# pangsu0613/TransCAR

Hardware: AMD Instinct MI355X
Metric: nuScenes frames/sec (6-cam+radar, 900 queries): fusion decoder (Detr3DHead.forward + box decode), FPN features resident in HBM (higher is better)
Workload: dtype f32 (linear steps and attention core of the batched launches: f16x2 split operands, 3 v_mfma_f32_16x16x32_f16 products, fp32 accumulate; activations of the 32-row tiles held as two f16 planes; 4- / 8-row tiles: f32 MFMA)

## Files before the change

transcar_amd/csrc/head.hip:

```cpp
#include <math.h>
#include <stdarg.h>
#include <stdlib.h>
#include <string.h>

#include "kernels.hpp"

namespace tc {

static thread_local char g_err[512] = "";

void set_error(const char* fmt, ...) {
  va_list ap;
  va_start(ap, fmt);
  vsnprintf(g_err, sizeof(g_err), fmt, ap);
  va_end(ap);
}

int check_launch(const char* what) {
  hipError_t e = hipGetLastError();
  if (e != hipSuccess) {
    set_error("%s: %s", what, hipGetErrorString(e));
    return (int)e;
  }
  return 0;
// ... 55 lines not shown
                             int np = 1) {
  const int rows = B * Q;
  const int NL = ncams * feats->num_levels * np;
  TC_TRY(linear(query, C, aw, rows, C, NL, 0, ws.logits, NL, s, pos));
  CamSampleArgs c;
  c.feats = *feats; c.B = B; c.Q = Q; c.C = C; c.num_cams = ncams; c.num_points = np;
  c.lidar2img = l2i; c.ref = ref; c.logits = ws.logits;
  for (int i = 0; i < 6; ++i) c.pc[i] = pc[i];
  c.img_h = img_h; c.img_w = img_w; c.out = ws.sampled; c.vis = nullptr; c.pair_counter = pair_counter;
  TC_TRY(launch_cam_sample(c, s));
  TC_TRY(linear(ws.sampled, C, oproj, rows, C, C, 0, ws.t0, C, s, nullptr, query, C));
  TC_TRY(launch_posenc_l1(ref, 3, 1, pe.l0.w, pe.l0.b, pe.n1.g, pe.n1.b, ws.pe0, rows, s));
  return linear(ws.pe0, C, pe.l3, rows, C, C, 0, ws.pe1, C, s);
}

static int head_points(const tc_head_weights* w) { return w->num_points > 0 ? w->num_points : 1; }

static int check_dims(const tc_head_weights* w) {
  TC_REQUIRE(w != nullptr, "weights pointer is null");
  TC_REQUIRE(w->abi_version == TC_ABI_VERSION, "tc_head_weights.abi_version=%d, library=%d",
             w->abi_version, TC_ABI_VERSION);
  TC_REQUIRE(w->embed_dims == 256 && w->num_heads == 8, "embed_dims=%d num_heads=%d (256/8 supported)",
             w->embed_dims, w->num_heads);
  TC_REQUIRE(w->num_layers >= 1 && w->num_layers <= TC_MAX_LAYERS, "num_layers=%d", w->num_layers);
  TC_REQUIRE(w->num_radar_layers >= 0 && w->num_radar_layers <= TC_MAX_RADAR_LAYERS,
             "num_radar_layers=%d", w->num_radar_layers);
  TC_REQUIRE(w->num_levels == 4, "num_levels=%d (4 supported)", w->num_levels);
  TC_REQUIRE(w->num_points >= 0 && w->num_cams * w->num_levels * head_points(w) <= TC_MAX_CAM_LOGITS,
             "num_points=%d (num_cams * num_levels * num_points <= %d supported)", w->num_points, TC_MAX_CAM_LOGITS);
  TC_REQUIRE((w->ffn_dims & 31) == 0 && (w->radar_in_dims & 3) == 0, "ffn_dims/radar_in_dims alignment");
  return 0;
}

static int decoder_refines(const tc_head_weights* w, bool* refine) {
  const int L = w->num_layers;
  const bool r = L < 2 || w->layers[0].reg.l0.w != nullptr;
  for (int l = 1; l + 1 < L; ++l)
    TC_REQUIRE((w->layers[l].reg.l0.w != nullptr) == r,
               "layers[%d].reg is %s but layers[0].reg is %s: below the last layer the reg branches are all set (box "
               "refinement) or all NULL (none)", l, r ? "NULL" : "set", r ? "set" : "NULL");
  TC_REQUIRE(w->layers[L - 1].reg.l0.w != nullptr, "layers[%d].reg is NULL: the last layer's reg branch "
             "(reg_branches[-1]) is required with and without box refinement", L - 1);
  *refine = r;
  return 0;
}

struct HeadWs {
  float *pos, *x, *qk, *vt, *attn_o, *t0, *t1, *t2, *ffn_h, *logits, *sampled;
  float *init_ref, *inter_refs, *hs, *reg_tmp, *box_m;
  float *tp0, *tp1, *f0, *f1, *f2, *radar_feat, *kv, *qproj, *rattn, *cxy, *addref, *qf;
  float* kv3[TC_MAX_RADAR_LAYERS];
  int* hits;
  int *perm, *hitflag;
  int qpad;
};

static size_t head_ws_layout(const tc_head_weights* w, int B, int T, void* base, size_t cap,
                             HeadWs* out) {
  const int Q = w->num_query, C = w->embed_dims, F = w->ffn_dims, L = w->num_layers;
  const size_t rows = (size_t)B * Q, rt = (size_t)B * T;
  const int qpad = ((Q + 15) / 16) * 16;
  Arena a(base, cap);
  HeadWs h;
  h.qpad = qpad;
  h.pos = a.take<float>(rows * C); h.x = a.take<float>(rows * C);
  h.qk = a.take<float>(rows * 2 * C); h.vt = a.take<float>((size_t)B * C * qpad);
  h.attn_o = a.take<float>(rows * C);
  h.t0 = a.take<float>(rows * C); h.t1 = a.take<float>(rows * C); h.t2 = a.take<float>(rows * C);
  h.ffn_h = a.take<float>(rows * F);
  h.logits = a.take<float>(rows * w->num_cams * w->num_levels * head_points(w));
  h.sampled = a.take<float>(rows * C);
  h.init_ref = a.take<float>(rows * 3); h.inter_refs = a.take<float>((size_t)L * rows * 3);
  h.hs = a.take<float>((size_t)L * rows * C);
  h.reg_tmp = a.take<float>(rows * w->code_size); h.box_m = a.take<float>(rows * w->code_size);
  h.tp0 = a.take<float>(rt * C); h.tp1 = a.take<float>(rt * C);
  h.f0 = a.take<float>(rt * 64); h.f1 = a.take<float>(rt * 128); h.f2 = a.take<float>(rt * C);
  h.radar_feat = a.take<float>(rt * C); h.kv = a.take<float>(rt * 2 * C);
  for (int i = 0; i < TC_MAX_RADAR_LAYERS; ++i) h.kv3[i] = a.take<float>(rt * 2 * C);
  h.qproj = a.take<float>(rows * C); h.rattn = a.take<float>(rows * C);
  h.cxy = a.take<float>(rows * 2); h.addref = a.take<float>(rows * 3);
  h.qf = a.take<float>(rows * C);
  h.hits = a.take<int>((size_t)TC_MAX_RADAR_LAYERS * rows);
  h.perm = a.take<int>(rows); h.hitflag = a.take<int>(rows);
  if (out) *out = h;
  return a.off;
}

static int head_forward_fused(const tc_head_weights* w, const tc_feats_nhwc* feats, int B,
                              const float* lidar2img, float img_h, float img_w,
                              const float* radar_tokens, int T, int pad_mult, float* all_cls_scores,
                              float* all_bbox_preds, const tc_head_aux* aux, const tc_head_options& opt,
                              const HeadWs& h_, hipStream_t s) {
  const int Q = w->num_query, C = w->embed_dims, L = w->num_layers, H = w->num_heads;
  const int code = w->code_size, ncls = w->num_classes;
  const int rows = B * Q, rt = B * T;
  const float attn_qscale = 1.4426950408889634f / sqrtf((float)(C / H));
  HeadWs h = h_;
  if (aux != nullptr) {
    if (aux->inter_states) h.hs = aux->inter_states;
    if (aux->inter_references) h.inter_refs = aux->inter_references;
    if (aux->last_box) h.box_m = aux->last_box;
  }
  unsigned long long* pairs = aux ? aux->sample_pairs : nullptr;
  const bool radar = w->num_radar_layers > 0;
  bool refine = true;
  TC_TRY(decoder_refines(w, &refine));

  const int enc_first = opt.phase != 0 && L > 1 ? L - 2 : 0;
  const int lid_begin = opt.phase == 2 ? enc_first : 0, lid_end = opt.phase == 1 ? enc_first : L;
  RadarEncodeArgs re;
  if (radar) {
    re.tokens = radar_tokens; re.RI = w->radar_in_dims; re.M = rt;
    re.rpe = w->radar_position_encoder; re.f0 = w->radar_feat0; re.f2 = w->radar_feat2;
    re.f4 = w->radar_feat4; re.nlayers = w->num_radar_layers;
    for (int r = 0; r < TC_MAX_RADAR_LAYERS; ++r) {
      const tc_mha& m = w->radar[r].attn;
      re.kvproj[r] = tc_linear{m.in_proj.w ? m.in_proj.w + (size_t)C * C : nullptr,
                               m.in_proj.b ? m.in_proj.b + C : nullptr};
      re.kv[r] = h.kv3[r];
    }
    re.radar_feat = h.radar_feat;
    re.w16_delta = w->packed16_delta; re.matrix_path = opt.matrix_path; re.range_status = opt.range_status;
  }

  const bool ddrop = opt.decoder_dropout_p > 0.0f;
  TC_REQUIRE(!ddrop || (unsigned long long)(opt.dropout_seed_stride ? 1 : B) * H * Q * Q < (1ull << 32),
             "decoder dropout: B*H*Q*Q exceeds 32 bits");
  if (radar && ddrop && opt.phase != 1) TC_TRY(launch_radar_encode(re, s));
  const bool folded = !ddrop && w->l0_attn_out != nullptr && w->l0_init_reference != nullptr;
  if (!folded && opt.phase != 2) {
    PrologueArgs pa;
    pa.qe = w->query_embedding; pa.Q = Q; pa.M = rows; pa.refpts = w->reference_points;
    pa.in_proj = w->layers[0].self_attn.in_proj; pa.init_ref = h.init_ref; pa.qk = h.qk; pa.vt = h.vt;
    pa.qpad = h.qpad; pa.qscale = attn_qscale; pa.w16_delta = w->packed16_delta;
    TC_TRY(launch_prologue(pa, s));
  }
  for (int lid = lid_begin; lid < lid_end; ++lid) {
    const bool l0c = folded && lid == 0;
    const bool init_in = lid == 0 || !refine;
    const float* ref_in = init_in ? (folded ? w->l0_init_reference : h.init_ref)
                                  : h.inter_refs + (size_t)(lid - 1) * rows * 3;
    DecoderChainArgs d;
    if (ddrop) {
      d.drop = make_drop(opt.decoder_dropout_p, opt.dropout_seed, 16u + 8u * (unsigned)lid, 0u);
      if (opt.dropout_seed_stride != 0) { d.drop.seed_stride = opt.dropout_seed_stride; d.drop.rows_per_sample = (unsigned)Q; }
    }
    d.attn_o = l0c ? w->l0_attn_out : h.attn_o;
    d.attn_mod = l0c ? Q : 0; d.ref_mod = folded && init_in ? Q : 0;
    if (lid == 0) { d.x_in = w->query_embedding + C; d.x_ld = 2 * C; d.x_mod = Q; }
    else { d.x_in = h.hs + (size_t)(lid - 1) * rows * C; d.x_ld = C; d.x_mod = 0; }
    d.qe = w->query_embedding; d.Q = Q;
    d.ref_in = ref_in; d.ref_out = h.inter_refs + (size_t)lid * rows * 3;
    d.box_m = lid == L - 1 ? h.box_m : nullptr;
    if (!refine) d.ref_out = h.addref;
    d.w = &w->layers[lid];
    d.next_in_proj = lid + 1 < L ? &w->layers[lid + 1].self_attn.in_proj : nullptr;
    d.qscale = attn_qscale;
    d.hs = h.hs + (size_t)lid * rows * C; d.qk = h.qk; d.vt = h.vt; d.qpad = h.qpad;
    d.cam.feats = *feats; d.cam.B = B; d.cam.Q = Q; d.cam.C = C; d.cam.num_cams = w->num_cams;
    d.cam.num_points = head_points(w);
    d.cam.lidar2img = lidar2img; d.cam.ref = ref_in; d.cam.logits = nullptr;
    for (int i = 0; i < 6; ++i) d.cam.pc[i] = w->pc_range[i];
    d.cam.img_h = img_h; d.cam.img_w = img_w; d.cam.out = nullptr; d.cam.vis = nullptr;
    d.cam.pair_counter = pairs;
    d.code = code; d.M = rows; d.tile_rows = opt.chain_tile_rows; d.matrix_path = opt.matrix_path;
    d.range_status = opt.range_status;
    if (!l0c) {
      const int trows = opt.chain_tile_rows ? opt.chain_tile_rows : (rows <= 1024 ? 4 : rows <= 2048 ? 8 : 16);
      if (trows >= 16 && opt.matrix_path != TC_MATRIX_F32) {
        PreGatherArgs pga;
        const bool pre = !ddrop && opt.cam_pregather == 1;
        if (pre) {
          float* pbuf = static_cast<float*>(opt.cam_pregather_ws);
          int* pmask = reinterpret_cast<int*>(pbuf + (size_t)rows * w->num_cams * w->num_levels * C);
          pga.cam = d.cam; pga.M = rows; pga.ref_mod = d.ref_mod; pga.out = pbuf; pga.mask = pmask;
          d.pre = pbuf; d.premask = pmask;
        }
        TC_TRY(launch_self_attn_core_x(h.qk, h.qk + C, 2 * C, h.vt, h.qpad, h.attn_o, C, B, Q, H, s, ddrop ? &d.drop : nullptr,
                                       pre ? &pga : nullptr));
      } else {
        TC_TRY(launch_self_attn_core(h.qk, h.qk + C, 2 * C, h.vt, h.qpad, h.attn_o, C, B, Q, H, s, ddrop ? &d.drop : nullptr));
      }
    }
    if (radar && !ddrop && lid == enc_first) TC_TRY(launch_decoder_chain_with_encoders(d, re, L > 1 ? 1 : 0, s));
    else if (radar && !ddrop && L > 1 && lid == enc_first + 1) TC_TRY(launch_decoder_chain_with_encoders(d, re, 2, s));
    else TC_TRY(launch_decoder_chain(d, s));
  }
  if (opt.phase == 1) return 0;
  if (!refine)
    TC_TRY(launch_ref_broadcast(folded ? w->l0_init_reference : h.init_ref, folded ? Q : 0, h.inter_refs, rows, L, s));
  if (aux) {
    if (aux->init_reference) {
      if (folded) {
        for (int b = 0; b < B; ++b)
          TC_HIP(hipMemcpyAsync(aux->init_reference + (size_t)b * Q * 3, w->l0_init_reference,
                                (size_t)Q * 3 * 4, hipMemcpyDeviceToDevice, s));
      } else {
        TC_HIP(hipMemcpyAsync(aux->init_reference, h.init_ref, (size_t)rows * 3 * 4, hipMemcpyDeviceToDevice, s));
      }
    }
  }
  if (!radar) return 0;
  RadarChainArgs rc;
  rc.qf = h.hs + (size_t)(L - 1) * rows * C;
  rc.ref_last = h.inter_refs + (size_t)(L - 1) * rows * 3;
  rc.box_m = h.box_m; rc.tokens = radar_tokens; rc.RI = w->radar_in_dims;
  for (int r = 0; r < TC_MAX_RADAR_LAYERS; ++r) { rc.kv[r] = h.kv3[r]; rc.w[r] = w->radar[r]; }
  rc.nlayers = w->num_radar_layers; rc.Q = Q; rc.T = T; rc.pad_mult = pad_mult; rc.code = code;
  rc.ncls = ncls; rc.M = rows; rc.qscale = 1.0f / sqrtf((float)(C / H));
  for (int i = 0; i < 6; ++i) rc.pc[i] = w->pc_range[i];
  rc.all_cls = all_cls_scores; rc.all_box = all_bbox_preds; rc.hits = h.hits;
  rc.tile_rows = opt.chain_tile_rows; rc.last_cls_only = opt.last_level_cls_only; rc.matrix_path = opt.matrix_path;
  rc.range_status = opt.range_status;
  if (opt.radar_row_order == 2 || (opt.radar_row_order == 0 && rows > 1024)) {
    TC_TRY(launch_radar_compact(rc.ref_last, rc.box_m, code, 0, w->pc_range, radar_tokens, w->radar_in_dims, B, Q, T,
                                w->radar[0].radius_min, w->radar[0].radius_max, h.hitflag, h.perm, s));
    rc.row_perm = h.perm;
  }
  TC_TRY(launch_radar_chain(rc, s));
  if (aux && aux->radar_hit_counts)
    TC_HIP(hipMemcpyAsync(aux->radar_hit_counts, h.hits, (size_t)w->num_radar_layers * rows * 4,
                          hipMemcpyDeviceToDevice, s));
  return 0;
}

struct PackItem { const float* src; int N, K; const float** slot; bool narrow; bool absent; };

static int collect_pack_items(const tc_head_weights* w, tc_head_weights* v, PackItem* it) {
  const int C = w->embed_dims, F = w->ffn_dims, NL = w->num_cams * w->num_levels * head_points(w);
  const int code = w->code_size, ncls = w->num_classes;
  int n = 0;
  auto add = [&](const tc_linear& src, tc_linear& dst, int N, int K, bool narrow = false, bool absent = false) {
// ... 175 lines not shown
size_t tc_self_attn_workspace_bytes(int B, int Q, int C) {
  const size_t rows = (size_t)B * Q;
  const size_t qpad = ((Q + 15) / 16) * 16;
  return arena_slice(rows * 2 * C, 4) + arena_slice((size_t)B * C * qpad, 4) + arena_slice(rows * C, 4);
}

int tc_self_attn_fwd(const tc_mha* w, const float* x, const float* pos, float* out, int B, int Q,
                     int C, int num_heads, void* workspace, size_t workspace_bytes,
                     tc_stream_t stream) {
  TC_REQUIRE(C == 256 && num_heads == 8, "self_attn: C=%d heads=%d (256/8 supported)", C, num_heads);
  TC_REQUIRE(workspace_bytes >= tc_self_attn_workspace_bytes(B, Q, C), "self_attn: workspace too small");
  const size_t rows = (size_t)B * Q;
  const int qpad = ((Q + 15) / 16) * 16;
  Arena a(workspace, workspace_bytes);
  float* qk = a.take<float>(rows * 2 * C);
  float* vt = a.take<float>((size_t)B * C * qpad);
  float* ao = a.take<float>(rows * C);
  return self_attn(*w, x, pos, out, B, Q, C, num_heads, qk, vt, qpad, ao, as_stream(stream));
}

int tc_decoder_layer_tail_fwd(const tc_decoder_layer* layer, const tc_linear* next_in_proj,
                              const tc_feats_nhwc* feats, int B, int Q, int num_cams,
                              int code_size, const float* attn_o, const float* x_in,
                              const float* query_embedding, const float* lidar2img,
                              const float* ref_in, const float* pc_range, float img_h,
                              float img_w, float* hs, float* ref_out, float* qk, float* vt,
                              int qpad, int tile_rows, tc_stream_t stream) {
  TC_REQUIRE(layer != nullptr && feats != nullptr, "decoder_layer_tail: null argument");
  const int C = 256;
  DecoderChainArgs d;
  d.attn_o = attn_o; d.x_in = x_in; d.x_ld = C; d.x_mod = 0;
  d.qe = query_embedding; d.Q = Q; d.ref_in = ref_in; d.ref_out = ref_out; d.box_m = nullptr;
  d.w = layer; d.next_in_proj = next_in_proj;
  d.qscale = 1.4426950408889634f / sqrtf(32.0f);
  d.hs = hs; d.qk = qk; d.vt = vt; d.qpad = qpad;
  d.cam.feats = *feats; d.cam.B = B; d.cam.Q = Q; d.cam.C = C; d.cam.num_cams = num_cams;
  d.cam.lidar2img = lidar2img; d.cam.ref = ref_in; d.cam.logits = nullptr;
  for (int i = 0; i < 6; ++i) d.cam.pc[i] = pc_range[i];
  d.cam.img_h = img_h; d.cam.img_w = img_w; d.cam.out = nullptr; d.cam.vis = nullptr;
  d.cam.pair_counter = nullptr;
  d.code = code_size; d.M = B * Q; d.tile_rows = TC_TILE_ROWS(tile_rows); d.matrix_path = TC_TILE_MATRIX(tile_rows);
  TC_REQUIRE(d.matrix_path <= TC_MATRIX_F16X2 && (tile_rows >> 10) == 0, "decoder_layer_tail: tile_rows=0x%x", tile_rows);
  TC_TRY(launch_decoder_chain(d, as_stream(stream)));
  if (layer->reg.l0.w == nullptr)
    TC_HIP(hipMemcpyAsync(ref_out, ref_in, (size_t)B * Q * 3 * 4, hipMemcpyDeviceToDevice, as_stream(stream)));
  return 0;
}

int tc_sdpa_fwd(const float* q, const float* k, int ld, const float* vt, int ldt, float* out, int ldo,
                int B, int Q, int num_heads, tc_stream_t stream) {
  return launch_self_attn_core(q, k, ld, vt, ldt, out, ldo, B, Q, num_heads, as_stream(stream));
}

size_t tc_sdpa_f16x2_workspace_bytes(int, int, int) { return 0; }

int tc_sdpa_fwd_f16x2(const float* qk, const float* vt, int ldt, float* out, int ldo, int B, int Q, int num_heads,
                      void* workspace, size_t workspace_bytes, tc_stream_t stream) {
  (void)workspace; (void)workspace_bytes;
  return launch_self_attn_core_x(qk, qk + num_heads * 32, 2 * num_heads * 32, vt, ldt, out, ldo, B, Q, num_heads, as_stream(stream));
}

size_t tc_radar_xattn_workspace_bytes(int B, int Q, int T, int C) {
  return arena_slice((size_t)B * T * 2 * C, 4) + 2 * arena_slice((size_t)B * Q * C, 4) +
         arena_slice((size_t)B * Q, 4);
}

int tc_radar_gated_xattn_fwd(const tc_mha* w, const float* query, const float* centre_xy,
                             const float* box, int code_size, const float* radar_feat,
                             const float* radar_xy, int B, int Q, int T, int C, int num_heads,
                             int pad_mult, float radius_min, float radius_max, float* out,
                             int* hit_counts, void* workspace, size_t workspace_bytes,
                             tc_stream_t stream) {
  TC_REQUIRE(C == 256 && num_heads == 8, "radar_xattn: C=%d heads=%d (256/8 supported)", C, num_heads);
  TC_REQUIRE(workspace_bytes >= tc_radar_xattn_workspace_bytes(B, Q, T, C), "radar_xattn: workspace too small");
  hipStream_t s = as_stream(stream);
  const int rows = B * Q, rt = B * T;
  Arena a(workspace, workspace_bytes);
  float* kv = a.take<float>((size_t)rt * 2 * C);
  float* qproj = a.take<float>((size_t)rows * C);
  float* rattn = a.take<float>((size_t)rows * C);
  int* hits = hit_counts ? hit_counts : a.take<int>(rows);
  tc_linear wkv{w->in_proj.w + (size_t)C * C, w->in_proj.b + C};
  TC_TRY(linear(radar_feat, C, wkv, rt, C, 2 * C, 0, kv, 2 * C, s));
  GemmArgs g;
  g.X = query; g.ldx = C; g.W = w->in_proj.w; g.ldw = C; g.bias = w->in_proj.b;
  g.Y = qproj; g.ldy = C; g.M = rows; g.K = C; g.N = C;
  g.scale = 1.0f / sqrtf((float)(C / num_heads)); g.scale_cols = C;
  TC_TRY(launch_gemm(g, s));
  RadarAttnArgs r;
  r.qproj = qproj; r.ldq = C; r.kv = kv; r.ldkv = 2 * C; r.centre_xy = centre_xy; r.ld_c = 2;
  r.box = box; r.code = code_size; r.radar_xy = radar_xy; r.ld_xy = 2;
  r.B = B; r.Q = Q; r.T = T; r.C = C; r.H = num_heads; r.pad_mult = pad_mult;
  r.rmin = radius_min; r.rmax = radius_max; r.attn_out = rattn; r.hit_counts = hits;
  TC_TRY(launch_radar_attn(r, s));
  return linear(rattn, C, w->out_proj, rows, C, C, 0, out, C, s, nullptr, query, C, hits);
}

static int read_options(const tc_head_options* options, tc_head_options& opt) {
  memset(&opt, 0, sizeof(opt));
  if (options != nullptr) opt = *options;
  TC_REQUIRE(opt.radar_row_order >= 0 && opt.radar_row_order <= 2, "options.radar_row_order=%d (0 automatic, 1 own order, 2 hits first)",
             opt.radar_row_order);
  TC_REQUIRE(opt.chain_tile_rows == 0 || opt.chain_tile_rows == 4 || opt.chain_tile_rows == 8 ||
                 opt.chain_tile_rows == 16 || opt.chain_tile_rows == 32,
             "options.chain_tile_rows=%d (0 = automatic, 4, 8, 16 or 32)", opt.chain_tile_rows);
  TC_REQUIRE(opt.chain_tile_rows != 32 || opt.matrix_path != TC_MATRIX_F32,
             "options.chain_tile_rows=32 exists on the f16x2 matrix path only (matrix_path = f32 was asked for)");
  TC_REQUIRE(opt.decoder_dropout_p >= 0.0f && opt.decoder_dropout_p < 1.0f, "options.decoder_dropout_p=%g",
             (double)opt.decoder_dropout_p);
  TC_REQUIRE(opt.phase >= 0 && opt.phase <= 2, "options.phase=%d (0 whole forward, 1 before the radar tokens, 2 the rest)",
             opt.phase);
  TC_REQUIRE(opt.phase == 0 || !opt.unfused, "options.phase=%d needs the fused path", opt.phase);
// ... 474 lines not shown
```

transcar_amd/csrc/kernels.hpp:

```cpp
#pragma once
#include "common.hpp"
#include "../../include/transcar_hip.h"

namespace tc {

struct GemmArgs {
  const float* X = nullptr;  int ldx = 0;
  const float* X2 = nullptr; int x2_cols = 0;
  const float* W = nullptr;  int ldw = 0;
  const float* bias = nullptr;
  const float* R = nullptr;  int ldr = 0;
  const int* rowgate = nullptr;
  float* Y = nullptr;        int ldy = 0;
  float* Yt = nullptr;
  int t_col0 = 0, t_ld = 0, t_rows_per_batch = 1;
  int M = 0, K = 0, N = 0;
  int act = 0;
  float scale = 1.0f; int scale_cols = 0;
};
int launch_gemm(const GemmArgs& a, hipStream_t s);

struct LnArgs {
  const float* a = nullptr;
  const float* b = nullptr;
// ... 84 lines not shown
  const float* qf; const float* ref_last; const float* box_m;
  const float* tokens; int RI;
  const float* kv[TC_MAX_RADAR_LAYERS];
  tc_radar_layer w[TC_MAX_RADAR_LAYERS];
  int nlayers, Q, T, pad_mult, code, ncls, M;
  float qscale; float pc[6];
  float* all_cls; float* all_box; int* hits;
  int tile_rows = 0;
  int matrix_path = 0;
  int last_cls_only = 0;
  int cen_from_box = 0;
  const int* row_perm = nullptr;
  float* const* tape = nullptr; size_t tape_stride = 0, hits_stride = 0;
  DropK drop = DropK{0, 0, 1.0f, 0, 1500, 0, 0, 0};
  int* range_status = nullptr;
};
enum DySlot { DY_DBOX = 0, DY_DT1, DY_DT0, DY_DC2, DY_DC0, DY_DFF, DY_DH, DY_DPROJ, DY_DQP, DY_DCLS, DY_COUNT };
struct RadarBwdChainArgs {
  tc_radar_layer wT[TC_MAX_RADAR_LAYERS];
  tc_radar_layer w[TC_MAX_RADAR_LAYERS];
  tc_radar_layer grads[TC_MAX_RADAR_LAYERS];
  const float* kv[TC_MAX_RADAR_LAYERS]; float* dkv[TC_MAX_RADAR_LAYERS];
  const float* cxy[TC_MAX_RADAR_LAYERS]; int ld_c[TC_MAX_RADAR_LAYERS]; const float* box[TC_MAX_RADAR_LAYERS];
  float* const* tape; size_t tape_stride, hits_stride; const int* hits;
  float* const* dy; size_t dy_stride;
  const float* d_cls; const float* d_box;
  const float* loss_vals = nullptr;
  float* loss_out = nullptr;
  const float* tokens; int RI, T, pad_mult;
  int nlayers, Q, M, code, ncls;
  float qscale;
  DropK drop;
  int tile_rows = 0;
  const DetAcc* det_device = nullptr;
};
int launch_radar_chain_bwd(const RadarBwdChainArgs& a, hipStream_t s);
enum TapeSlot { TS_QP = 0, TS_AO, TS_X1, TS_X2, TS_H, TS_SUM, TS_X3, TS_C0, TS_C1, TS_C2, TS_C3, TS_T0, TS_T1, TS_TREG,
                TS_U0, TS_U1, TS_U2, TS_POS, TS_F0, TS_F1, TS_F2, TS_MEM, TS_COUNT };
int launch_radar_chain(const RadarChainArgs& a, hipStream_t s);

int launch_radar_compact(const float* ref_last, const float* box, int code, int cen_from_box,
                         const float* pc6_host, const float* tokens, int RI, int B, int Q, int T,
                         float rmin, float rmax, int* flags, int* perm, hipStream_t s);

int launch_gate_selfcheck(int n_radii, unsigned long long seed, unsigned long long* mismatches, hipStream_t s);
int launch_rowops_selfcheck(int n_blocks, unsigned long long seed, unsigned long long* mismatches, hipStream_t s);

int launch_self_attn_core(const float* q, const float* k, int ld, const float* vt, int ldt,
                          float* out, int ldo, int B, int Q, int H, hipStream_t s,
                          const DropK* drop = nullptr);
struct PreGatherArgs {
  CamSampleArgs cam; int M, ref_mod; float* out; int* mask;
};
int launch_self_attn_core_x(const float* q, const float* k, int ld, const float* vt, int ldt, float* out, int ldo,
                            int B, int Q, int H, hipStream_t s, const DropK* drop = nullptr,
                            const PreGatherArgs* pregather = nullptr);

struct RadarAttnArgs {
  const float* qproj; int ldq;
  const float* kv; int ldkv;
  const float* centre_xy; int ld_c;
  const float* box; int code;
  const float* radar_xy; int ld_xy;
  int B, Q, T, C, H, pad_mult;
  float rmin, rmax;
  float* attn_out;
  int* hit_counts;
  float qscale = 1.0f;
  DropK drop = DropK{0, 0, 1.0f, 0, 1500, 0, 0, 0};
};
int launch_radar_attn(const RadarAttnArgs& a, hipStream_t s);
int launch_dropout(const float* x, const float* res, const int* gate, int rows, int cols, const DropK& d,
                   float* out, hipStream_t s);

int launch_linear_bwd_data(const float* dy, const float* relu_out, const int* row_gate,
                           const float* w, const float* in_relu_mask, float* dx, int M, int K,
                           int N, float alpha, int accumulate, hipStream_t s);
int launch_linear_bwd_weight(const float* x, const float* dy, const float* relu_out,
                             const int* row_gate, float* dw, float* db, int M, int K, int N,
                             float alpha, hipStream_t s);
struct WeightJob { const float* x; const float* dy; float* dw; float* db; int M, K, N; const float* relu = nullptr;
                   int ldx = 0;  };
int launch_linear_bwd_weight_group(const WeightJob* jobs, int n, hipStream_t s);
DetAcc& current_det();
DetAcc*& current_det_device();
struct DetScope {
  DetAcc saved; DetAcc* saved_dev;
  DetScope(const DetAcc& d, DetAcc* dev) : saved(current_det()), saved_dev(current_det_device()) { current_det() = d; current_det_device() = dev; }
  ~DetScope() { current_det() = saved; current_det_device() = saved_dev; }
  DetScope(const DetScope&) = delete;
  DetScope& operator=(const DetScope&) = delete;
};
int launch_det_flush(const DetAcc& d, int range, hipStream_t s);
int launch_det_store(const DetAcc& d, DetAcc* dst, hipStream_t s);
int launch_ln256_bwd(const float* a, const float* b, const float* gamma, const float* dy,
                     const float* relu_out, float* dz, float* dgamma, float* dbeta, int M,
                     hipStream_t s);
int launch_radar_attn_bwd(const RadarAttnArgs& a, float qscale, const float* d_attn, float* dq,
                          float* dkv, hipStream_t s);
int launch_box_ref_bwd(const float* d_box, int code, float* d_prev, int M, hipStream_t s);
int launch_sqnorm(const float* g, size_t n, float* out, hipStream_t s);
int launch_adamw(float* p, const float* g, float* m, float* v, size_t n, float lr, float b1,
                 float b2, float eps, float wd, int step, float grad_scale, float max_norm,
                 const float* sqnorm, hipStream_t s);

size_t packed_floats(int N, int K);
int launch_pack_linear(const float* W, int N, int K, float* P, float* P16, float* PH, hipStream_t s);
struct PackJob { const float* W; float* P; float* P16; int N, K; int transpose = 0, ldw = 0; float* PH = nullptr; };
int launch_pack_group(const PackJob* jobs, int n, hipStream_t s);
// ... 23 lines not shown
```

transcar_amd/csrc/self_attn.hip:

```cpp
#include <string.h>

#include "kernels.hpp"
#include "rowdev.hpp"

namespace tc {

#define MFMA4(a, b, c) __builtin_amdgcn_mfma_f32_16x16x4f32((a), (b), (c), 0, 0, 0)

constexpr int SA_NW = 8;
constexpr float SA_TAU = 8.0f;

__device__ __forceinline__ float max_lanes_16_32(float x) {
  float a = x, b = x;
  asm volatile("s_nop 1\n\tv_permlane32_swap_b32 %0, %1\n\ts_nop 1\n\tv_max_f32 %0, %0, %1\n\tv_mov_b32 %1, %0\n\ts_nop 1\n\t"
               "v_permlane16_swap_b32 %0, %1\n\ts_nop 1\n\tv_max_f32 %0, %0, %1"
               : "+v"(a), "+v"(b));
  return a;
}

struct KVFrag { float4 ka, kb, v0, v1; };

struct KVPtr { const float* k; const float* v0; const float* v1; };

__device__ __forceinline__ KVFrag load_kv(const KVPtr& p) {
// ... 241 lines not shown
      const float alpha = first ? 1.0f : __builtin_amdgcn_exp2f(-delta);
#pragma unroll
      for (int pp = 0; pp < NP; ++pp)
#pragma unroll
        for (int i = 0; i < 8; ++i) sc[pp][u][i] -= delta;
      st[u].o0 *= alpha; st[u].o1 *= alpha; st[u].lsum *= alpha; st[u].l *= alpha;
      st[u].negm -= delta;
    }
  }
  const unsigned one2 = 0x3C003C00u;
  const float4 ones = make_float4(__uint_as_float(one2), __uint_as_float(one2), __uint_as_float(one2), __uint_as_float(one2));
  (void)ones;
#pragma unroll
  for (int pp = 0; pp < NP; ++pp) {
    const float4 v0h = fb[pp][4][lane], v0l = fb[pp][5][lane], v1h = fb[pp][6][lane], v1l = fb[pp][7][lane];
#pragma unroll
    for (int u = 0; u < QT; ++u) {
      float p[8];
#pragma unroll
      for (int i = 0; i < 8; ++i) p[i] = __builtin_amdgcn_exp2f(sc[pp][u][i]);
      if (!SX_L_MFMA) st[u].l += ((p[0] + p[1]) + (p[2] + p[3])) + ((p[4] + p[5]) + (p[6] + p[7]));
      if constexpr (DROP) {
        const unsigned idx = dbase[u] + key0 + 32u * (unsigned)pp;
        const unsigned m0 = drop_keep4(drop->seed, drop->site, idx, drop->thr), m1 = drop_keep4(drop->seed, drop->site, idx + 4u, drop->thr);
#pragma unroll
        for (int i = 0; i < 4; ++i) {
          p[i] = ((m0 >> i) & 1u) ? p[i] * drop->scale : 0.0f;
          p[4 + i] = ((m1 >> i) & 1u) ? p[4 + i] * drop->scale : 0.0f;
        }
      }
      float4 p_h, p_l;
#ifdef SX_NO_PLO
      {
        unsigned hh[4];
#pragma unroll
        for (int i = 0; i < 4; ++i) hh[i] = sa_pk(p[2 * i], p[2 * i + 1]);
        p_h = make_float4(__uint_as_float(hh[0]), __uint_as_float(hh[1]), __uint_as_float(hh[2]), __uint_as_float(hh[3]));
        p_l = p_h;
      }
#else
      sx_split1(p, p_h, p_l);
#endif
      st[u].o0 = MFMAH(v0h, p_h, st[u].o0); st[u].o1 = MFMAH(v1h, p_h, st[u].o1);
      if (SX_L_MFMA) st[u].lsum = MFMAH(ones, p_h, st[u].lsum);
      st[u].o0 = MFMAH(v0l, p_h, st[u].o0); st[u].o1 = MFMAH(v1l, p_h, st[u].o1);
#ifndef SX_NO_PLO
      st[u].o0 = MFMAH(v0h, p_l, st[u].o0); st[u].o1 = MFMAH(v1h, p_l, st[u].o1);
      if (SX_L_MFMA) st[u].lsum = MFMAH(ones, p_l, st[u].lsum);
#endif
    }
  }
}

template <int QT, bool DROP = false>
__global__ __launch_bounds__(SX_NW * 64) __attribute__((amdgpu_waves_per_eu(SX_OCC, SX_OCC))) void self_attn_x_kernel(
    const float* __restrict__ q, const float* __restrict__ k, int ld, const float* __restrict__ vt, int ldt,
    float* __restrict__ out, int ldo, int Q, int C, int H, int BH, DropK drop, PreGatherK pg) {
  constexpr int QW = 16 * QT * SX_NW;
  __shared__ float4 frag[2][SX_CP][8][64];
  const int tid = threadIdx.x, lane = tid & 63, wave = __builtin_amdgcn_readfirstlane(tid >> 6);
  if constexpr (!DROP) {
    const int nattn = (int)gridDim.x - pg.nblocks;
    if ((int)blockIdx.x >= nattn) {
      const int r0 = ((int)blockIdx.x - nattn) * SX_PG_ROWS + wave * (SX_PG_ROWS / SX_NW);
      cam_pregather_rows<4>(pg, r0, SX_PG_ROWS / SX_NW, lane);
      return;
    }
  }
  const int r = lane & 15, g = lane >> 4;
  const int Gf = Q / QW, nfull = BH * Gf;
  int bh, qg;
  {
    const int idx = blockIdx.x;
    if (idx >= nfull) { bh = idx - nfull; qg = Gf; }
    else if ((BH & 7) == 0) { const int slot = idx >> 3; bh = (slot / Gf) * 8 + (idx & 7); qg = slot % Gf; }
    else { bh = idx / Gf; qg = idx % Gf; }
  }
  const int b = bh / H, h = bh - b * H;
  const size_t brow = (size_t)b * Q;
  const int q0 = qg * QW + wave * 16 * QT;
  const bool active = q0 < Q;
  constexpr int NT = SX_NW * 64, TPT = NT >= 256 ? 1 : 256 / NT;
  const bool stager = tid < 256;
  bool is_k[TPT];
  int gg[TPT], rowi[TPT], dfrag[TPT], dlane[TPT];
  const float* src[TPT];
#pragma unroll
  for (int tk = 0; tk < TPT; ++tk) {
    const int t = tid + tk * NT;
    is_k[tk] = __builtin_amdgcn_readfirstlane(t) < 128;
    const int tt = t & 127;
    gg[tk] = tt & 3; rowi[tk] = tt >> 2;
    dfrag[tk] = is_k[tk] ? 2 * ((rowi[tk] >> 2) & 1) : 4 + 2 * (rowi[tk] >> 4);
    dlane[tk] = is_k[tk] ? 16 * gg[tk] + 4 * (rowi[tk] >> 3) + (rowi[tk] & 3) : 16 * gg[tk] + (rowi[tk] & 15);
    src[tk] = is_k[tk] ? k + brow * ld + h * 32 + 8 * gg[tk] : vt + ((size_t)b * C + h * 32 + rowi[tk]) * ldt + 8 * gg[tk];
  }
  const float4 zero4 = make_float4(0.f, 0.f, 0.f, 0.f);
  auto fetch = [&](int j, int tk, float4& x0, float4& x1) {
    const int key0 = 32 * j;
    if (is_k[tk]) {
      const float* p = src[tk] + (size_t)min(key0 + rowi[tk], Q - 1) * ld;
      x0 = ld4(p); x1 = ld4(p + 4);
    } else {
      const int kk = key0 + 8 * gg[tk];
      const float* p = src[tk] + key0;
      x0 = kk + 3 < ldt ? ld4(p) : zero4;
      x1 = kk + 7 < ldt ? ld4(p + 4) : zero4;
      if (kk + 7 >= Q) {
        if (kk + 0 >= Q) x0.x = 0.f;
        if (kk + 1 >= Q) x0.y = 0.f;
        if (kk + 2 >= Q) x0.z = 0.f;
        if (kk + 3 >= Q) x0.w = 0.f;
        if (kk + 4 >= Q) x1.x = 0.f;
        if (kk + 5 >= Q) x1.y = 0.f;
        if (kk + 6 >= Q) x1.z = 0.f;
        if (kk + 7 >= Q) x1.w = 0.f;
      }
    }
  };
  auto put = [&](int buf, int pp, int tk, const float4& x0, const float4& x1) {
    float4 hi, lo;
    sx_split(x0, x1, hi, lo);
    frag[buf][pp][dfrag[tk]][dlane[tk]] = hi;
    frag[buf][pp][dfrag[tk] + 1][dlane[tk]] = lo;
  };
  const int np = (Q + 31) >> 5, nchunk = (np + SX_CP - 1) / SX_CP;
  float4 x[SX_CP][TPT][2];
  if (stager) {
#pragma unroll
    for (int pp = 0; pp < SX_CP; ++pp)
#pragma unroll
      for (int tk = 0; tk < TPT; ++tk)
        if (pp < np) fetch(pp, tk, x[pp][tk][0], x[pp][tk][1]);
  }
  float4 q_h[QT], q_l[QT];
  SXState st[QT];
  unsigned dbase[QT];
  if (DROP) drop.seed += (unsigned long long)b * drop.seed_stride;
#pragma unroll
  for (int u = 0; u < QT; ++u) {
    const int qrow = min(q0 + 16 * u + r, Q - 1);
    dbase[u] = DROP ? (((drop.rows_per_sample ? 0u : (unsigned)b) * (unsigned)H + (unsigned)h) * (unsigned)Q + (unsigned)qrow) * (unsigned)Q + 8u * (unsigned)g : 0u;
    const float* qp = q + (brow + qrow) * ld + h * 32 + 8 * g;
#ifdef SX_Q_NT
    sx_split(ldg4_stream(qp), ldg4_stream(qp + 4), q_h[u], q_l[u]);
#else
    sx_split(ld4(qp), ld4(qp + 4), q_h[u], q_l[u]);
#endif
    st[u].o0 = st[u].o1 = st[u].lsum = st[u].negm = f32x4{0.f, 0.f, 0.f, 0.f};
    st[u].l = 0.0f;
  }
  if (stager) {
#pragma unroll
    for (int pp = 0; pp < SX_CP; ++pp)
#pragma unroll
      for (int tk = 0; tk < TPT; ++tk)
        if (pp < np) put(0, pp, tk, x[pp][tk][0], x[pp][tk][1]);
  }
  __syncthreads();
#pragma unroll 1
  for (int c = 0; c < nchunk; ++c) {
    const int buf = c & 1;
#ifdef SX_NO_STAGE
    const bool more = false;
#else
    const bool more = c + 1 < nchunk;
#endif
    if (more && stager) {
#pragma unroll
      for (int pp = 0; pp < SX_CP; ++pp)
#pragma unroll
        for (int tk = 0; tk < TPT; ++tk)
          if ((c + 1) * SX_CP + pp < np) fetch((c + 1) * SX_CP + pp, tk, x[pp][tk][0], x[pp][tk][1]);
    }
    __builtin_amdgcn_sched_barrier(0);
#ifndef SX_NO_COMPUTE
    if (active) {
      const int left = np - c * SX_CP;
      const int nvalid_last = min(32, Q - 32 * (c * SX_CP + min(left, SX_CP) - 1));
      static_assert(SX_CP == 2, "the chunk dispatch below is written for two pairs");
      const unsigned key0 = 32u * (unsigned)(c * SX_CP);
      if (SX_NPC == 2 && left >= 2) sx_chunk<QT, 2, DROP>(frag[buf], lane, g, q_h, q_l, st, c == 0, nvalid_last, &drop, dbase, key0);
      else {
        sx_chunk<QT, 1, DROP>(frag[buf], lane, g, q_h, q_l, st, c == 0, left >= 2 ? 32 : nvalid_last, &drop, dbase, key0);
        if (left >= 2) sx_chunk<QT, 1, DROP>(frag[buf] + 1, lane, g, q_h, q_l, st, false, nvalid_last, &drop, dbase, key0 + 32u);
      }
    }
#endif
    __builtin_amdgcn_sched_barrier(0);
    if (more && stager) {
#pragma unroll
      for (int pp = 0; pp < SX_CP; ++pp)
#pragma unroll
        for (int tk = 0; tk < TPT; ++tk)
          if ((c + 1) * SX_CP + pp < np) put(buf ^ 1, pp, tk, x[pp][tk][0], x[pp][tk][1]);
    }
    __syncthreads();
  }
  if (!active) return;
#pragma unroll
  for (int u = 0; u < QT; ++u) {
    const int qrow = q0 + 16 * u + r;
    if (qrow < Q) {
      float l = st[u].lsum[0];
      if (!SX_L_MFMA) { l = st[u].l; l += __shfl_xor(l, 16); l += __shfl_xor(l, 32); }
      const float inv = 1.0f / l;
      float* op = out + (brow + qrow) * ldo + h * 32 + 4 * g;
      st4(op, make_float4(st[u].o0[0] * inv, st[u].o0[1] * inv, st[u].o0[2] * inv, st[u].o0[3] * inv));
      st4(op + 16, make_float4(st[u].o1[0] * inv, st[u].o1[1] * inv, st[u].o1[2] * inv, st[u].o1[3] * inv));
    }
  }
}

void fill_camk(const CamSampleArgs& a, CamK& p);

int launch_self_attn_core_x(const float* q, const float* k, int ld, const float* vt, int ldt, float* out, int ldo,
                            int B, int Q, int H, hipStream_t s, const DropK* drop, const PreGatherArgs* pregather) {
  TC_REQUIRE(Q > 0 && B > 0 && H > 0, "self_attn(f16x2): empty problem");
  TC_REQUIRE((ldt & 3) == 0 && ldt >= ((Q + 15) / 16) * 16, "self_attn(f16x2): ldt=%d too small for Q=%d", ldt, Q);
  constexpr int QT = SX_QT_VALUE, QW = 16 * QT * SX_NW;
  const int BH = B * H, Gf = Q / QW, G = (Q + QW - 1) / QW;
  const int nattn = BH * Gf + (G > Gf ? BH : 0);
  PreGatherK pg;
  memset(&pg, 0, sizeof(pg));
  if (drop != nullptr && drop->thr != 0) {
    TC_REQUIRE(pregather == nullptr, "self_attn(f16x2): the pre-gather rides in eval launches only");
    TC_REQUIRE((unsigned long long)(drop->rows_per_sample ? 1 : B) * H * Q * Q < (1ull << 32),
               "self_attn(f16x2): dropout index space (B*H*Q*Q) exceeds 32 bits");
    hipLaunchKernelGGL((self_attn_x_kernel<QT, true>), dim3(nattn), dim3(SX_NW * 64), 0, s, q, k, ld, vt, ldt, out, ldo, Q, H * 32, H, BH, *drop, pg);
  } else {
    if (pregather != nullptr) {
      const PreGatherArgs& a = *pregather;
      TC_REQUIRE(a.out != nullptr && a.mask != nullptr && a.M > 0, "self_attn(f16x2): pre-gather buffers");
      TC_REQUIRE(a.cam.C == 256 && a.cam.feats.num_levels == 4 && a.cam.num_cams <= 8, "self_attn(f16x2): pre-gather shape");
      for (int l = 0; l < a.cam.feats.num_levels; ++l)
        TC_REQUIRE((long long)a.cam.B * a.cam.num_cams * a.cam.feats.H[l] * a.cam.feats.W[l] < (1ll << 31),
                   "self_attn(f16x2): pre-gather level %d has too many pixels for one call", l);
      fill_camk(a.cam, pg.cam);
      pg.cam.vis = nullptr; pg.cam.out = nullptr; pg.cam.pair_counter = nullptr; pg.cam.logits = nullptr;
      pg.M = a.M; pg.ref_mod = a.ref_mod; pg.out = a.out; pg.mask = a.mask;
      pg.nblocks = (a.M + SX_PG_ROWS - 1) / SX_PG_ROWS;
    }
    hipLaunchKernelGGL((self_attn_x_kernel<QT, false>), dim3(nattn + pg.nblocks), dim3(SX_NW * 64), 0, s, q, k, ld, vt, ldt, out, ldo, Q, H * 32, H, BH,
                       DropK{0, 0, 1.0f, 0, 0, 0, 0, 0}, pg);
  }
  return check_launch("self_attn(f16x2, staged)");
}

int launch_self_attn_core(const float* q, const float* k, int ld, const float* vt, int ldt,
                          float* out, int ldo, int B, int Q, int H, hipStream_t s, const DropK* drop) {
  TC_REQUIRE(Q > 0 && B > 0 && H > 0, "self_attn: empty problem");
  TC_REQUIRE((ldt & 3) == 0 && ldt >= ((Q + 15) / 16) * 16, "self_attn: ldt=%d too small for Q=%d", ldt, Q);
  constexpr int QT = 2;
  dim3 grid((Q + 16 * QT - 1) / (16 * QT), H, B);
  if (drop != nullptr && drop->thr != 0) {
    TC_REQUIRE((unsigned long long)(drop->rows_per_sample ? 1 : B) * H * Q * Q < (1ull << 32),
               "self_attn: dropout index space (B*H*Q*Q) exceeds 32 bits");
    hipLaunchKernelGGL((self_attn_kernel<QT, true>), grid, dim3(SA_NW * 64), 0, s, q, k, ld, vt, ldt, out, ldo, Q,
                       H * 32, *drop);
  } else {
    hipLaunchKernelGGL((self_attn_kernel<QT, false>), grid, dim3(SA_NW * 64), 0, s, q, k, ld, vt, ldt, out, ldo, Q,
                       H * 32, DropK{0, 0, 1.0f, 0, 0, 0, 0, 0});
  }
  return check_launch("self_attn");
}

}
```

Before: 10250.

## Pre-split K/V into f16 plane image and DMA it straight into LDS

Adds a small kernel that converts the K and V^T tiles of each batch-head once into hi/lo f16 fragment planes laid out exactly as the attention kernel's shared-memory fragments. The attention kernel then copies these planes into LDS with global_load_lds_dwordx4, replacing the per-block register staging, split and LDS store. This avoids repeating the K/V fetch and split in every query-group block. The cost is an extra launch, a workspace buffer, and a full write and read of the plane image.

Result: no change. 10300, median of 6 (+0.5%).

```diff
diff --git a/transcar_amd/csrc/head.hip b/transcar_amd/csrc/head.hip
--- a/transcar_amd/csrc/head.hip
+++ b/transcar_amd/csrc/head.hip
@@ -131,6 +131,7 @@
   float* kv3[TC_MAX_RADAR_LAYERS];
   int* hits;
   int *perm, *hitflag;
+  void* kvp;
   int qpad;
 };
 
@@ -161,6 +162,7 @@
   h.qf = a.take<float>(rows * C);
   h.hits = a.take<int>((size_t)TC_MAX_RADAR_LAYERS * rows);
   h.perm = a.take<int>(rows); h.hitflag = a.take<int>(rows);
+  h.kvp = a.take<char>(sx_plane_bytes(B, Q, w->num_heads));
   if (out) *out = h;
   return a.off;
 }
@@ -256,7 +258,7 @@
           d.pre = pbuf; d.premask = pmask;
         }
         TC_TRY(launch_self_attn_core_x(h.qk, h.qk + C, 2 * C, h.vt, h.qpad, h.attn_o, C, B, Q, H, s, ddrop ? &d.drop : nullptr,
-                                       pre ? &pga : nullptr));
+                                       pre ? &pga : nullptr, h.kvp));
       } else {
         TC_TRY(launch_self_attn_core(h.qk, h.qk + C, 2 * C, h.vt, h.qpad, h.attn_o, C, B, Q, H, s, ddrop ? &d.drop : nullptr));
       }
@@ -538,12 +540,14 @@
   return launch_self_attn_core(q, k, ld, vt, ldt, out, ldo, B, Q, num_heads, as_stream(stream));
 }
 
-size_t tc_sdpa_f16x2_workspace_bytes(int, int, int) { return 0; }
+size_t tc_sdpa_f16x2_workspace_bytes(int B, int Q, int num_heads) { return sx_plane_bytes(B, Q, num_heads); }
 
 int tc_sdpa_fwd_f16x2(const float* qk, const float* vt, int ldt, float* out, int ldo, int B, int Q, int num_heads,
                       void* workspace, size_t workspace_bytes, tc_stream_t stream) {
-  (void)workspace; (void)workspace_bytes;
-  return launch_self_attn_core_x(qk, qk + num_heads * 32, 2 * num_heads * 32, vt, ldt, out, ldo, B, Q, num_heads, as_stream(stream));
+  TC_REQUIRE(workspace == nullptr || (B > 0 && Q > 0 && num_heads > 0 && workspace_bytes >= sx_plane_bytes(B, Q, num_heads)),
+             "sdpa(f16x2): workspace of %zu bytes too small", workspace_bytes);
+  return launch_self_attn_core_x(qk, qk + num_heads * 32, 2 * num_heads * 32, vt, ldt, out, ldo, B, Q, num_heads, as_stream(stream),
+                                 nullptr, nullptr, workspace);
 }
 
 size_t tc_radar_xattn_workspace_bytes(int B, int Q, int T, int C) {
diff --git a/transcar_amd/csrc/kernels.hpp b/transcar_amd/csrc/kernels.hpp
--- a/transcar_amd/csrc/kernels.hpp
+++ b/transcar_amd/csrc/kernels.hpp
@@ -160,9 +160,10 @@
 struct PreGatherArgs {
   CamSampleArgs cam; int M, ref_mod; float* out; int* mask;
 };
+size_t sx_plane_bytes(int B, int Q, int H);
 int launch_self_attn_core_x(const float* q, const float* k, int ld, const float* vt, int ldt, float* out, int ldo,
                             int B, int Q, int H, hipStream_t s, const DropK* drop = nullptr,
-                            const PreGatherArgs* pregather = nullptr);
+                            const PreGatherArgs* pregather = nullptr, void* planes = nullptr);
 
 struct RadarAttnArgs {
   const float* qproj; int ldq;
diff --git a/transcar_amd/csrc/self_attn.hip b/transcar_amd/csrc/self_attn.hip
--- a/transcar_amd/csrc/self_attn.hip
+++ b/transcar_amd/csrc/self_attn.hip
@@ -317,10 +317,67 @@
   }
 }
 
-template <int QT, bool DROP = false>
+struct SXTask { const float* src; int rowi, gg, dfrag, dlane; bool is_k; };
+__device__ __forceinline__ SXTask sx_task(int t, const float* k, int ld, const float* vt, int ldt, int b, int Q, int C, int h) {
+  SXTask r;
+  r.is_k = __builtin_amdgcn_readfirstlane(t) < 128;
+  const int tt = t & 127;
+  r.gg = tt & 3; r.rowi = tt >> 2;
+  r.dfrag = r.is_k ? 2 * ((r.rowi >> 2) & 1) : 4 + 2 * (r.rowi >> 4);
+  r.dlane = r.is_k ? 16 * r.gg + 4 * (r.rowi >> 3) + (r.rowi & 3) : 16 * r.gg + (r.rowi & 15);
+  r.src = r.is_k ? k + (size_t)b * Q * ld + h * 32 + 8 * r.gg : vt + ((size_t)b * C + h * 32 + r.rowi) * ldt + 8 * r.gg;
+  return r;
+}
+__device__ __forceinline__ void sx_fetch(const SXTask& t, int j, int Q, int ld, int ldt, float4& x0, float4& x1) {
+  const int key0 = 32 * j;
+  if (t.is_k) {
+    const float* p = t.src + (size_t)min(key0 + t.rowi, Q - 1) * ld;
+    x0 = ld4(p); x1 = ld4(p + 4);
+  } else {
+    const float4 zero4 = make_float4(0.f, 0.f, 0.f, 0.f);
+    const int kk = key0 + 8 * t.gg;
+    const float* p = t.src + key0;
+    x0 = kk + 3 < ldt ? ld4(p) : zero4;
+    x1 = kk + 7 < ldt ? ld4(p + 4) : zero4;
+    if (kk + 7 >= Q) {
+      if (kk + 0 >= Q) x0.x = 0.f;
+      if (kk + 1 >= Q) x0.y = 0.f;
+      if (kk + 2 >= Q) x0.z = 0.f;
+      if (kk + 3 >= Q) x0.w = 0.f;
+      if (kk + 4 >= Q) x1.x = 0.f;
+      if (kk + 5 >= Q) x1.y = 0.f;
+      if (kk + 6 >= Q) x1.z = 0.f;
+      if (kk + 7 >= Q) x1.w = 0.f;
+    }
+  }
+}
+
+constexpr int SX_PAIR_F4 = 8 * 64;
+size_t sx_plane_bytes(int B, int Q, int H) { return (size_t)B * H * ((Q + 31) / 32) * SX_PAIR_F4 * sizeof(float4); }
+
+__global__ __launch_bounds__(256) void sx_planes_kernel(const float* __restrict__ k, int ld, const float* __restrict__ vt, int ldt,
+                                                        float4* __restrict__ planes, int Q, int C, int H) {
+  const int j = blockIdx.x, bh = blockIdx.y, b = bh / H, h = bh - b * H;
+  const SXTask t = sx_task(threadIdx.x, k, ld, vt, ldt, b, Q, C, h);
+  float4 x0, x1, hi, lo;
+  sx_fetch(t, j, Q, ld, ldt, x0, x1);
+  sx_split(x0, x1, hi, lo);
+  float4* d = planes + ((size_t)bh * gridDim.x + j) * SX_PAIR_F4;
+  d[t.dfrag * 64 + t.dlane] = hi;
+  d[(t.dfrag + 1) * 64 + t.dlane] = lo;
+}
+
+__device__ __forceinline__ void sx_glds16(const void* gsrc, const void* lds) {
+  unsigned keep;
+  const unsigned dst = (unsigned)(size_t)lds;
+  asm volatile("s_mov_b32 %0, m0\n\ts_mov_b32 m0, %2\n\ts_nop 0\n\tglobal_load_lds_dwordx4 %1, off\n\ts_mov_b32 m0, %0"
+               : "=&s"(keep) : "v"(gsrc), "s"(dst) : "memory");
+}
+
+template <int QT, bool DROP, bool PLANES>
 __global__ __launch_bounds__(SX_NW * 64) __attribute__((amdgpu_waves_per_eu(SX_OCC, SX_OCC))) void self_attn_x_kernel(
     const float* __restrict__ q, const float* __restrict__ k, int ld, const float* __restrict__ vt, int ldt,
-    float* __restrict__ out, int ldo, int Q, int C, int H, int BH, DropK drop, PreGatherK pg) {
+    const float4* __restrict__ planes, float* __restrict__ out, int ldo, int Q, int C, int H, int BH, DropK drop, PreGatherK pg) {
   constexpr int QW = 16 * QT * SX_NW;
   __shared__ float4 frag[2][SX_CP][8][64];
   const int tid = threadIdx.x, lane = tid & 63, wave = __builtin_amdgcn_readfirstlane(tid >> 6);
@@ -345,58 +402,35 @@
   const size_t brow = (size_t)b * Q;
   const int q0 = qg * QW + wave * 16 * QT;
   const bool active = q0 < Q;
-  constexpr int NT = SX_NW * 64, TPT = NT >= 256 ? 1 : 256 / NT;
-  const bool stager = tid < 256;
-  bool is_k[TPT];
-  int gg[TPT], rowi[TPT], dfrag[TPT], dlane[TPT];
-  const float* src[TPT];
-#pragma unroll
-  for (int tk = 0; tk < TPT; ++tk) {
-    const int t = tid + tk * NT;
-    is_k[tk] = __builtin_amdgcn_readfirstlane(t) < 128;
-    const int tt = t & 127;
-    gg[tk] = tt & 3; rowi[tk] = tt >> 2;
-    dfrag[tk] = is_k[tk] ? 2 * ((rowi[tk] >> 2) & 1) : 4 + 2 * (rowi[tk] >> 4);
-    dlane[tk] = is_k[tk] ? 16 * gg[tk] + 4 * (rowi[tk] >> 3) + (rowi[tk] & 3) : 16 * gg[tk] + (rowi[tk] & 15);
-    src[tk] = is_k[tk] ? k + brow * ld + h * 32 + 8 * gg[tk] : vt + ((size_t)b * C + h * 32 + rowi[tk]) * ldt + 8 * gg[tk];
-  }
-  const float4 zero4 = make_float4(0.f, 0.f, 0.f, 0.f);
-  auto fetch = [&](int j, int tk, float4& x0, float4& x1) {
-    const int key0 = 32 * j;
-    if (is_k[tk]) {
-      const float* p = src[tk] + (size_t)min(key0 + rowi[tk], Q - 1) * ld;
-      x0 = ld4(p); x1 = ld4(p + 4);
-    } else {
-      const int kk = key0 + 8 * gg[tk];
-      const float* p = src[tk] + key0;
-      x0 = kk + 3 < ldt ? ld4(p) : zero4;
-      x1 = kk + 7 < ldt ? ld4(p + 4) : zero4;
-      if (kk + 7 >= Q) {
-        if (kk + 0 >= Q) x0.x = 0.f;
-        if (kk + 1 >= Q) x0.y = 0.f;
-        if (kk + 2 >= Q) x0.z = 0.f;
-        if (kk + 3 >= Q) x0.w = 0.f;
-        if (kk + 4 >= Q) x1.x = 0.f;
-        if (kk + 5 >= Q) x1.y = 0.f;
-        if (kk + 6 >= Q) x1.z = 0.f;
-        if (kk + 7 >= Q) x1.w = 0.f;
-      }
+  const int np = (Q + 31) >> 5, nchunk = (np + SX_CP - 1) / SX_CP;
+  static_assert(!PLANES || (SX_NW == 4 && SX_CP == 2), "the plane copy is written for four waves and two-pair chunks");
+  const char* img = reinterpret_cast<const char*>(planes + (size_t)bh * np * SX_PAIR_F4) + 16 * lane;
+  auto dma = [&](int c, int buf) {
+    if (SX_CP * c + (wave >> 1) < np) {
+#pragma unroll
+      for (int i = 0; i < 4; ++i)
+        sx_glds16(img + (size_t)(16 * c + 4 * wave + i) * 1024, reinterpret_cast<const char*>(&frag[buf][0][0][0]) + (4 * wave + i) * 1024);
     }
   };
+  constexpr int NT = SX_NW * 64, TPT = PLANES ? 1 : NT >= 256 ? 1 : 256 / NT;
+  const bool stager = !PLANES && tid < 256;
+  SXTask task[TPT];
+#pragma unroll
+  for (int tk = 0; tk < TPT; ++tk) task[tk] = sx_task(tid + tk * NT, k, ld, vt, ldt, b, Q, C, h);
   auto put = [&](int buf, int pp, int tk, const float4& x0, const float4& x1) {
     float4 hi, lo;
     sx_split(x0, x1, hi, lo);
-    frag[buf][pp][dfrag[tk]][dlane[tk]] = hi;
-    frag[buf][pp][dfrag[tk] + 1][dlane[tk]] = lo;
+    frag[buf][pp][task[tk].dfrag][task[tk].dlane] = hi;
+    frag[buf][pp][task[tk].dfrag + 1][task[tk].dlane] = lo;
   };
-  const int np = (Q + 31) >> 5, nchunk = (np + SX_CP - 1) / SX_CP;
   float4 x[SX_CP][TPT][2];
+  if constexpr (PLANES) dma(0, 0);
   if (stager) {
 #pragma unroll
     for (int pp = 0; pp < SX_CP; ++pp)
 #pragma unroll
       for (int tk = 0; tk < TPT; ++tk)
-        if (pp < np) fetch(pp, tk, x[pp][tk][0], x[pp][tk][1]);
+        if (pp < np) sx_fetch(task[tk], pp, Q, ld, ldt, x[pp][tk][0], x[pp][tk][1]);
   }
   float4 q_h[QT], q_l[QT];
   SXState st[QT];
@@ -407,11 +441,7 @@
     const int qrow = min(q0 + 16 * u + r, Q - 1);
     dbase[u] = DROP ? (((drop.rows_per_sample ? 0u : (unsigned)b) * (unsigned)H + (unsigned)h) * (unsigned)Q + (unsigned)qrow) * (unsigned)Q + 8u * (unsigned)g : 0u;
     const float* qp = q + (brow + qrow) * ld + h * 32 + 8 * g;
-#ifdef SX_Q_NT
-    sx_split(ldg4_stream(qp), ldg4_stream(qp + 4), q_h[u], q_l[u]);
-#else
     sx_split(ld4(qp), ld4(qp + 4), q_h[u], q_l[u]);
-#endif
     st[u].o0 = st[u].o1 = st[u].lsum = st[u].negm = f32x4{0.f, 0.f, 0.f, 0.f};
     st[u].l = 0.0f;
   }
@@ -422,24 +452,22 @@
       for (int tk = 0; tk < TPT; ++tk)
         if (pp < np) put(0, pp, tk, x[pp][tk][0], x[pp][tk][1]);
   }
+  if constexpr (PLANES) __builtin_amdgcn_s_waitcnt(0x0F70);
   __syncthreads();
 #pragma unroll 1
   for (int c = 0; c < nchunk; ++c) {
     const int buf = c & 1;
-#ifdef SX_NO_STAGE
-    const bool more = false;
-#else
     const bool more = c + 1 < nchunk;
-#endif
-    if (more && stager) {
+    if constexpr (PLANES) {
+      if (more) dma(c + 1, buf ^ 1);
+    } else if (more && stager) {
 #pragma unroll
       for (int pp = 0; pp < SX_CP; ++pp)
 #pragma unroll
         for (int tk = 0; tk < TPT; ++tk)
-          if ((c + 1) * SX_CP + pp < np) fetch((c + 1) * SX_CP + pp, tk, x[pp][tk][0], x[pp][tk][1]);
+          if ((c + 1) * SX_CP + pp < np) sx_fetch(task[tk], (c + 1) * SX_CP + pp, Q, ld, ldt, x[pp][tk][0], x[pp][tk][1]);
     }
     __builtin_amdgcn_sched_barrier(0);
-#ifndef SX_NO_COMPUTE
     if (active) {
       const int left = np - c * SX_CP;
       const int nvalid_last = min(32, Q - 32 * (c * SX_CP + min(left, SX_CP) - 1));
@@ -451,9 +479,10 @@
         if (left >= 2) sx_chunk<QT, 1, DROP>(frag[buf] + 1, lane, g, q_h, q_l, st, false, nvalid_last, &drop, dbase, key0 + 32u);
       }
     }
-#endif
     __builtin_amdgcn_sched_barrier(0);
-    if (more && stager) {
+    if constexpr (PLANES) {
+      if (more) __builtin_amdgcn_s_waitcnt(0x0F70);
+    } else if (more && stager) {
 #pragma unroll
       for (int pp = 0; pp < SX_CP; ++pp)
 #pragma unroll
@@ -480,21 +509,29 @@
 void fill_camk(const CamSampleArgs& a, CamK& p);
 
 int launch_self_attn_core_x(const float* q, const float* k, int ld, const float* vt, int ldt, float* out, int ldo,
-                            int B, int Q, int H, hipStream_t s, const DropK* drop, const PreGatherArgs* pregather) {
+                            int B, int Q, int H, hipStream_t s, const DropK* drop, const PreGatherArgs* pregather,
+                            void* planes) {
   TC_REQUIRE(Q > 0 && B > 0 && H > 0, "self_attn(f16x2): empty problem");
   TC_REQUIRE((ldt & 3) == 0 && ldt >= ((Q + 15) / 16) * 16, "self_attn(f16x2): ldt=%d too small for Q=%d", ldt, Q);
   constexpr int QT = SX_QT_VALUE, QW = 16 * QT * SX_NW;
   const int BH = B * H, Gf = Q / QW, G = (Q + QW - 1) / QW;
   const int nattn = BH * Gf + (G > Gf ? BH : 0);
+  float4* pl = static_cast<float4*>(planes);
+  if (pl != nullptr) {
+    TC_REQUIRE(BH <= 65535, "self_attn(f16x2): B * num_heads = %d exceeds the plane kernel's grid", BH);
+    hipLaunchKernelGGL(sx_planes_kernel, dim3((Q + 31) / 32, BH), dim3(256), 0, s, k, ld, vt, ldt, pl, Q, H * 32, H);
+  }
   PreGatherK pg;
   memset(&pg, 0, sizeof(pg));
   if (drop != nullptr && drop->thr != 0) {
     TC_REQUIRE(pregather == nullptr, "self_attn(f16x2): the pre-gather rides in eval launches only");
     TC_REQUIRE((unsigned long long)(drop->rows_per_sample ? 1 : B) * H * Q * Q < (1ull << 32),
                "self_attn(f16x2): dropout index space (B*H*Q*Q) exceeds 32 bits");
-    hipLaunchKernelGGL((self_attn_x_kernel<QT, true>), dim3(nattn), dim3(SX_NW * 64), 0, s, q, k, ld, vt, ldt, out, ldo, Q, H * 32, H, BH, *drop, pg);
+    TC_REQUIRE(pl != nullptr, "self_attn(f16x2): train-mode launches take the plane image");
+    hipLaunchKernelGGL((self_attn_x_kernel<QT, true, true>), dim3(nattn), dim3(SX_NW * 64), 0, s, q, k, ld, vt, ldt, pl, out, ldo, Q, H * 32, H, BH, *drop, pg);
   } else {
     if (pregather != nullptr) {
+      TC_REQUIRE(pl != nullptr, "self_attn(f16x2): the pre-gather rides in launches with the plane image");
       const PreGatherArgs& a = *pregather;
       TC_REQUIRE(a.out != nullptr && a.mask != nullptr && a.M > 0, "self_attn(f16x2): pre-gather buffers");
       TC_REQUIRE(a.cam.C == 256 && a.cam.feats.num_levels == 4 && a.cam.num_cams <= 8, "self_attn(f16x2): pre-gather shape");
@@ -506,10 +543,13 @@
       pg.M = a.M; pg.ref_mod = a.ref_mod; pg.out = a.out; pg.mask = a.mask;
       pg.nblocks = (a.M + SX_PG_ROWS - 1) / SX_PG_ROWS;
     }
-    hipLaunchKernelGGL((self_attn_x_kernel<QT, false>), dim3(nattn + pg.nblocks), dim3(SX_NW * 64), 0, s, q, k, ld, vt, ldt, out, ldo, Q, H * 32, H, BH,
-                       DropK{0, 0, 1.0f, 0, 0, 0, 0, 0}, pg);
-  }
-  return check_launch("self_attn(f16x2, staged)");
+    const DropK nodrop{0, 0, 1.0f, 0, 0, 0, 0, 0};
+    if (pl != nullptr)
+      hipLaunchKernelGGL((self_attn_x_kernel<QT, false, true>), dim3(nattn + pg.nblocks), dim3(SX_NW * 64), 0, s, q, k, ld, vt, ldt, pl, out, ldo, Q, H * 32, H, BH, nodrop, pg);
+    else
+      hipLaunchKernelGGL((self_attn_x_kernel<QT, false, false>), dim3(nattn + pg.nblocks), dim3(SX_NW * 64), 0, s, q, k, ld, vt, ldt, pl, out, ldo, Q, H * 32, H, BH, nodrop, pg);
+  }
+  return check_launch(pl != nullptr ? "self_attn(f16x2, planes)" : "self_attn(f16x2, staged)");
 }
 
 int launch_self_attn_core(const float* q, const float* k, int ld, const float* vt, int ldt,
```
